# yangdongchao/Text-to-sound-Synthesis

Hardware: AMD Instinct MI355X
Metric: 10s clips/sec whole-node, 100-step Diffsound sample + VQ decode + vocoder (higher is better)
Workload: dtype f32 via 2-way fp16 split (3 MFMA passes, fp32 accumulate); 1 GPU; BASELINE configs[2]: full pipeline, batch 64 per GPU, 100 diffusion steps, codebook 256: CLIP text tower -> 19-layer denoiser -> SpecVQGAN decode -> MelGAN 22 kHz; global_batch=64, n_layer=19, parallelism=caption-sharded x1

## Files before the change

text-to-sound-synthesis_amd/csrc/gemm_f16x2_ps.hip:

```cpp
#include <stdlib.h>

#include "common.h"


typedef _Float16 h8 __attribute__((ext_vector_type(8)));
typedef unsigned u32x4 __attribute__((ext_vector_type(4)));
typedef __attribute__((address_space(1))) const void* ds_gptr;
typedef __attribute__((address_space(3))) void* ds_lptr;

#define PS_HLD 32
#define PS_BM 288
#define PS_BN 256
#define PS_LEAD 6
#define PS_GM 4
#define PS_STAGE_BYTES (2 * 2 * (PS_BM + PS_BN) * PS_HLD * 2)
#define PS_VT_BYTES (2 * 2 * PS_BN * 36 * 4)
#define PS_LDS_BYTES (PS_VT_BYTES > PS_STAGE_BYTES ? PS_VT_BYTES : PS_STAGE_BYTES)
#define PS_SIG(q_) ((0x78 >> (2 * (q_))) & 3)

enum { PS_EPI_ROW = 0, PS_EPI_SPLIT = 1, PS_EPI_ATTN = 2 };

template <int EPI, bool NB16>
__global__ __launch_bounds__(512, 1) void ds_gemm_f16x2_ps_kernel(const GemmParams p) {
    extern __shared__ __attribute__((aligned(16))) unsigned char smem_raw[];
    constexpr int BM = PS_BM, BN = PS_BN, HLD = PS_HLD, LEAD = PS_LEAD;
    constexpr int APL = BM * HLD, BPL = BN * HLD, STAGE = 2 * (APL + BPL);
    _Float16* smem = (_Float16*)smem_raw;
    const int tid = threadIdx.x, lane = tid & 63, wave = tid >> 6, l31 = lane & 31, hh = lane >> 5;
    const int wr = wave >> 2, wc = wave & 3;
    const int L = p.rows_per_sample;
    const int tiles_n = p.N / BN, nblk = gridDim.x;
    int bid = blockIdx.x;
// ... 109 lines not shown
            e1[ks] = *(const h8*)(Ec + APL + swz[ks]);                                               \
        }                                                                                            \
    } while (0)
#define PS_READ_B(buf_, s_)                                                                          \
    do {                                                                                             \
        const _Float16* Bc = smem + (buf_) * STAGE + 2 * APL + (wc * 64 + (s_) * 32 + l31) * HLD;    \
        _Pragma("unroll") for (int ks = 0; ks < 2; ++ks) {                                           \
            b0[s_][ks] = *(const h8*)(Bc + swz[ks]);                                                 \
            b1[s_][ks] = *(const h8*)(Bc + BPL + swz[ks]);                                           \
        }                                                                                            \
    } while (0)
#define PS_QUAD(sa_, sb_)                                                                            \
    do {                                                                                             \
        _Pragma("unroll") for (int ks = 0; ks < 2; ++ks) {                                           \
            _Pragma("unroll") for (int ib = 0; ib < 2; ++ib)                                         \
                acc[2 * (sa_) + ib][sb_] = __builtin_amdgcn_mfma_f32_32x32x16_f16(a1[ks][ib], b0[sb_][ks], acc[2 * (sa_) + ib][sb_], 0, 0, 0); \
            _Pragma("unroll") for (int ib = 0; ib < 2; ++ib)                                         \
                acc[2 * (sa_) + ib][sb_] = __builtin_amdgcn_mfma_f32_32x32x16_f16(a0[ks][ib], b1[sb_][ks], acc[2 * (sa_) + ib][sb_], 0, 0, 0); \
            _Pragma("unroll") for (int ib = 0; ib < 2; ++ib)                                         \
                acc[2 * (sa_) + ib][sb_] = __builtin_amdgcn_mfma_f32_32x32x16_f16(a0[ks][ib], b0[sb_][ks], acc[2 * (sa_) + ib][sb_], 0, 0, 0); \
        }                                                                                            \
    } while (0)
#define PS_EXTRA(sb_)                                                                                \
    do {                                                                                             \
        _Pragma("unroll") for (int ks = 0; ks < 2; ++ks) {                                           \
            acc8 = __builtin_amdgcn_mfma_f32_32x32x16_f16(e1[ks], b0[sb_][ks], acc8, 0, 0, 0);       \
            acc8 = __builtin_amdgcn_mfma_f32_32x32x16_f16(e0[ks], b1[sb_][ks], acc8, 0, 0, 0);       \
            acc8 = __builtin_amdgcn_mfma_f32_32x32x16_f16(e0[ks], b0[sb_][ks], acc8, 0, 0, 0);       \
        }                                                                                            \
    } while (0)
#define PS_READ_EB16(buf_)                                                                           \
    do {                                                                                             \
        const _Float16* Bc = smem + (buf_) * STAGE + 2 * APL + ((2 * wc + wr) * 32 + l15) * HLD;     \
        _Pragma("unroll") for (int tt = 0; tt < 2; ++tt) {                                           \
            eb0[tt] = *(const h8*)(Bc + tt * 16 * HLD + swzq);                                       \
            eb1[tt] = *(const h8*)(Bc + BPL + tt * 16 * HLD + swzq);                                 \
        }                                                                                            \
    } while (0)
#define PS_READ_EA16(buf_)                                                                           \
    do {                                                                                             \
        const _Float16* Ec = smem + (buf_) * STAGE + (256 + l15) * HLD;                              \
        ea0 = *(const h8*)(Ec + swzq);                                                               \
        ea1 = *(const h8*)(Ec + APL + swzq);                                                         \
    } while (0)
#define PS_EXTRA16()                                                                                 \
    do {                                                                                             \
        _Pragma("unroll") for (int tt = 0; tt < 2; ++tt) {                                           \
            acc9[tt] = __builtin_amdgcn_mfma_f32_16x16x32_f16(ea1, eb0[tt], acc9[tt], 0, 0, 0);      \
            acc9[tt] = __builtin_amdgcn_mfma_f32_16x16x32_f16(ea0, eb1[tt], acc9[tt], 0, 0, 0);      \
            acc9[tt] = __builtin_amdgcn_mfma_f32_16x16x32_f16(ea0, eb0[tt], acc9[tt], 0, 0, 0);      \
        }                                                                                            \
    } while (0)
#define PS_PHASE(P, BUF)                                                                             \
    do {                                                                                             \
        if (P == 0) { PS_READ_A(BUF, 0); PS_READ_B(BUF, 0); }                                        \
        if (P == 1) { PS_READ_B(BUF, 1); if (NB16) PS_READ_EB16(BUF); }                              \
        if (P == 2) { PS_READ_A(BUF, 1); if (NB16) PS_READ_EA16(BUF); }                              \
        if (P == 3 && !NB16) PS_READ_E(BUF);                                                         \
        PS_FENCE();                                                                                  \
        {                                                                                            \
            constexpr int dq = (P) + LEAD;                                     \
            const int tq = t + (dq >> 2);                                                            \
            if (tq < nk) {                                                                           \
                PS_ISSUE_LOOP(tq, dq & 3, ((BUF) + (dq >> 2)) & 1);                                  \
                asm volatile("s_waitcnt vmcnt(9)" ::: "memory");    \
// ... 33 lines not shown
        PS_PHASE(0, 1); PS_PHASE(1, 1); PS_PHASE(2, 1); PS_PHASE(3, 1);
        --t;
    }
    if (wr == 0) PS_LBAR();
    asm volatile("s_waitcnt vmcnt(0)" ::: "memory");

    constexpr int WROW = 128, EROW0 = 256;
    constexpr bool HALF_TILE = false;
    const bool hasE = true;
    const int pos0 = 0, tile_rows = L;
#include "gemm_f16x2_ps_epilogue.inc"
}

#define PH_AROWS 144
#define PH_STAGE_BYTES (2 * (PH_AROWS + PS_BN) * PS_HLD * 2)
#define PH_LDS_BYTES (3 * PH_STAGE_BYTES > PS_VT_BYTES ? 3 * PH_STAGE_BYTES : PS_VT_BYTES)

template <int EPI>
__global__ __launch_bounds__(512, 1) void ds_gemm_f16x2_ph_kernel(const GemmParams p) {
    extern __shared__ __attribute__((aligned(16))) unsigned char smem_raw[];
    constexpr bool NB16 = true;
    constexpr int BN = PS_BN, HLD = PS_HLD;
    constexpr int APL = PH_AROWS * HLD, BPL = BN * HLD, STAGE = 2 * (APL + BPL);
    _Float16* smem = (_Float16*)smem_raw;
    const int tid = threadIdx.x, lane = tid & 63, wave = tid >> 6, l31 = lane & 31, hh = lane >> 5;
    const int wr = wave >> 2, wc = wave & 3;
    const int L = p.rows_per_sample;
    const int tiles_n = p.N / BN, nblk = gridDim.x;
    int bid = blockIdx.x;
    {
        const int xcd = bid & 7, idx = bid >> 3, q = nblk >> 3, r = nblk & 7;
// ... 103 lines not shown
        _Pragma("unroll") for (int tt = 0; tt < 2; ++tt) {                                           \
            eb0[tt] = *(const h8*)(Bc + tt * 16 * HLD + swzq);                                       \
            eb1[tt] = *(const h8*)(Bc + BPL + tt * 16 * HLD + swzq);                                 \
        }                                                                                            \
    } while (0)
#define PH_READ_EA16(st_)                                                                            \
    do {                                                                                             \
        const _Float16* Ec = smem + (st_) * STAGE + (128 + l15) * HLD;                               \
        ea0 = *(const h8*)(Ec + swzq);                                                               \
        ea1 = *(const h8*)(Ec + APL + swzq);                                                         \
    } while (0)
#define PH_QUAD(sb_)                                                                                 \
    do {                                                                                             \
        _Pragma("unroll") for (int ks = 0; ks < 2; ++ks) {                                           \
            _Pragma("unroll") for (int ib = 0; ib < 2; ++ib)                                         \
                acc[ib][sb_] = __builtin_amdgcn_mfma_f32_32x32x16_f16(a1[ks][ib], b0[sb_][ks], acc[ib][sb_], 0, 0, 0); \
            _Pragma("unroll") for (int ib = 0; ib < 2; ++ib)                                         \
                acc[ib][sb_] = __builtin_amdgcn_mfma_f32_32x32x16_f16(a0[ks][ib], b1[sb_][ks], acc[ib][sb_], 0, 0, 0); \
            _Pragma("unroll") for (int ib = 0; ib < 2; ++ib)                                         \
                acc[ib][sb_] = __builtin_amdgcn_mfma_f32_32x32x16_f16(a0[ks][ib], b0[sb_][ks], acc[ib][sb_], 0, 0, 0); \
        }                                                                                            \
    } while (0)
#define PH_EXTRA16()                                                                                 \
    do {                                                                                             \
        _Pragma("unroll") for (int tt = 0; tt < 2; ++tt) {                                           \
            acc9[tt] = __builtin_amdgcn_mfma_f32_16x16x32_f16(ea1, eb0[tt], acc9[tt], 0, 0, 0);      \
            acc9[tt] = __builtin_amdgcn_mfma_f32_16x16x32_f16(ea0, eb1[tt], acc9[tt], 0, 0, 0);      \
            acc9[tt] = __builtin_amdgcn_mfma_f32_16x16x32_f16(ea0, eb0[tt], acc9[tt], 0, 0, 0);      \
        }                                                                                            \
    } while (0)
#define PH_PHASE(P, ST)                                                                              \
    do {                                                                                             \
        if (P == 0) { PH_READ_A(ST); PH_READ_B(ST, 0); if (hasE && wr == 0) PH_READ_EB16(ST); }      \
        else { PH_READ_B(ST, 1); if (hasE) { PH_READ_EA16(ST); if (wr == 1) PH_READ_EB16(ST); } }    \
        PS_FENCE();                                                                                  \
        if (tt + 2 < nk) {                                                                           \
            PH_ISSUE_LOOP(P, ((ST) + 2) % 3);                                                        \
            if (P == 0) asm volatile("s_waitcnt vmcnt(11)" ::: "memory");    \
            else asm volatile("s_waitcnt vmcnt(10)" ::: "memory");           \
        } else {                                                                                     \
            asm volatile("s_waitcnt vmcnt(0)" ::: "memory");     \
        }                                                                                            \
        PS_BAR();                                                                                    \
// ... 28 lines not shown
        if (t + 1 < nk) { const int tt = t + 1; PH_PHASE(0, 1); PH_PHASE(1, 1); }
        if (t + 2 < nk) { const int tt = t + 2; PH_PHASE(0, 2); PH_PHASE(1, 2); }
    }
    if (wr == 0) PS_BAR();
    asm volatile("s_waitcnt vmcnt(0)" ::: "memory");
    constexpr int WROW = 64, EROW0 = 128;
    constexpr bool HALF_TILE = true;
#include "gemm_f16x2_ps_epilogue.inc"
}

static bool ps_serves(const GemmParams& p, bool half) {
    const int L = p.rows_per_sample;
    if (!p.a_split || L <= 0 || L > PS_BM - 15 || L <= 240 || p.M % L != 0) return false;
    if (half && L != PS_BM - 16) return false;
    if (p.N % PS_BN != 0 || p.K % 64 != 0 || p.lda != p.K || p.ldw != p.K) return false;
    if (p.store == DS_STORE_ROW && !p.c_split) {
        if (((p.N | p.ldc | p.ldr) & 3) != 0 || (((uintptr_t)p.C | (uintptr_t)p.R) & 15) != 0) return false;
    } else if (p.store == DS_STORE_ROW) {
        if (p.R) return false;
    } else if (p.store == DS_STORE_ATTN) {
        if (p.row_off != 0 || p.attn_heads * 64 % PS_BN != 0) return false;
    } else {
        return false;
    }
    return true;
}

int ds_gemm_f16x2_ps_choice(long B, long N, bool half_ok) {
    const long tf = B * (N / PS_BN), th = 2 * tf;
    const double ef = (double)tf / (double)(((tf + 255) / 256) * 256);
// ... 64 lines not shown
```

text-to-sound-synthesis_amd/csrc/gemm_f16x2_ps_epilogue.inc:

```
    int tid_e = tid;
    asm volatile("" : "+v"(tid_e));
    const int l31e = tid_e & 31, hhe = (tid_e >> 5) & 1, wre = tid_e >> 8, wce = (tid_e >> 6) & 3;
    const int off = row_lo - m0;
    int vhi = off + tile_rows;
    if (vhi > p.M - m0) vhi = p.M - m0;
    const float osc = p.out_scale;
    constexpr bool ALLV = NB16;
    const int qe = (tid_e >> 4) & 3, ne = tid_e & 15;
    const int cl0 = (wce * 2 + 0) * 32 + l31e, cl1 = (wce * 2 + 1) * 32 + l31e;
    const int cl9 = (wce * 2 + wre) * 32 + (NB16 ? PS_SIG(ne >> 2) * 4 + (ne & 3) : l31e);
    float bv0 = 0.f, bv1 = 0.f, bv9a = 0.f, bv9b = 0.f;
    if (p.bias) {
        bv0 = p.bias[n0 + cl0]; bv1 = p.bias[n0 + cl1]; bv9a = p.bias[n0 + cl9];
        if (NB16) bv9b = p.bias[n0 + cl9 + 16];
    }
    constexpr int EBUF = 64 * BN;
#define PS_TROW(S, rs_) ((S) < 4 ? ((rs_) >> 5) * WROW + (S) * 32 + ((rs_) & 31) : EROW0 + (rs_))
#define PS_STEP_VALUES(S, GELU, STORE)                                                               \
    do {                                                                                             \
        if ((S) < 4) {                                                                               \
            _Pragma("unroll") for (int j = 0; j < 2; ++j) {                                          \
                const int cl = j ? cl1 : cl0;                                                        \
                const float bv = j ? bv1 : bv0;                                                      \
                _Pragma("unroll") for (int r = 0; r < 16; ++r) {                                     \
                    float v = acc[(S) < 4 ? (S) : 0][j][r] * osc + bv;                               \
                    if (GELU) v = ds_gelu2_fast(v);                                                  \
                    STORE(wre * 32 + (r & 3) + 8 * (r >> 2) + 4 * hhe, cl, v);                       \
                }                                                                                    \
            }                                                                                        \
        } else if (NB16) {                                                                           \
            _Pragma("unroll") for (int tt = 0; tt < 2; ++tt)                                         \
                _Pragma("unroll") for (int r = 0; r < 4; ++r) {                                      \
                    float v = acc9[tt][r] * osc + (tt ? bv9b : bv9a);                                \
                    if (GELU) v = ds_gelu2_fast(v);                                                  \
                    STORE(4 * PS_SIG(qe) + r, cl9 + tt * 16, v);                                     \
                }                                                                                    \
        } else {                                                                                     \
            _Pragma("unroll") for (int r = 0; r < 16; ++r) {                                         \
                float v = acc8[r] * osc + bv9a;                                                      \
                if (GELU) v = ds_gelu2_fast(v);                                                      \
                STORE((r & 3) + 8 * (r >> 2) + 4 * hhe, cl9, v);                                     \
            }                                                                                        \
        }                                                                                            \
    } while (0)
    const bool gelu = p.act == DS_ACT_GELU2;
    __syncthreads();

    if constexpr (EPI == PS_EPI_ROW) {
#define PS_ST_F32(rs_, cl_, v_) Tf[(rs_) * BN + (cl_)] = (v_)
#define PS_ROW_ITERS(S) (((S) < 4 ? 64 : (NB16 ? 16 : 32)) / 8)
#define PS_ROW_CONST(S, it) ((S) < 4 ? ((it) >> 2) * WROW + (S) * 32 + 8 * ((it) & 3) : EROW0 + 8 * (it))
#define PS_ROW_LOAD(S, res_, HASR)                                                                   \
    do {                                                                                             \
        _Pragma("unroll") for (int it = 0; it < PS_ROW_ITERS(S); ++it) {                             \
            res_[it] = f32x4{0.f, 0.f, 0.f, 0.f};                                                    \
            if (ALLV) {                                                                              \
                if (HASR) res_[it] = *(const f32x4*)(p.R + (size_t)(m0 + PS_ROW_CONST(S, it)) * p.ldr + n0 + voR); \
            } else {                                                                                 \
                const int trow = PS_TROW(S, (tid_e >> 6) + 8 * it);                                  \
                if ((HASR) && trow >= off && trow < vhi)                                             \
                    res_[it] = *(const f32x4*)(p.R + (size_t)(m0 + trow) * p.ldr + n0 + (tid_e & 63) * 4); \
            }                                                                                        \
        }                                                                                            \
    } while (0)
#define PS_ROW_STAGE(S, res_, HASR)                                                                    \
    do {                                                                                             \
        float* Tf = (float*)smem_raw + ((S) & 1) * EBUF;                                             \
        if (!AHEAD) PS_ROW_LOAD(S, res_, HASR);                                                      \
        if (gelu) PS_STEP_VALUES(S, true, PS_ST_F32); else PS_STEP_VALUES(S, false, PS_ST_F32);      \
    } while (0)
#define PS_ROW_STORE(S, res_)                                                                        \
    do {                                                                                             \
        const float* Tf = (const float*)smem_raw + ((S) & 1) * EBUF;                                 \
        const int cc = tid_e & 63, col = n0 + cc * 4;                                                \
        __syncthreads();                                                                             \
        _Pragma("unroll") for (int it = 0; it < PS_ROW_ITERS(S); ++it) {                             \
            const int rs = (tid_e >> 6) + 8 * it, trow = PS_TROW(S, rs);                             \
            if (ALLV || (trow >= off && trow < vhi)) {                                               \
                const f32x4 vv_ = *(const f32x4*)(Tf + rs * BN + cc * 4) + res_[it];                 \
                if (ALLV) *(f32x4*)(p.C + (size_t)(m0 + PS_ROW_CONST(S, it)) * p.ldc + n0 + voC) = vv_; \
                else *(f32x4*)(p.C + (size_t)(m0 + trow) * p.ldc + col) = vv_;                       \
            }                                                                                        \
        }                                                                                            \
    } while (0)
#define PS_ROW_STEP(S, res_, HASR) do { PS_ROW_STAGE(S, res_, HASR); PS_ROW_STORE(S, res_); } while (0)
        f32x4 resA[8], resB[8];
        constexpr bool AHEAD = ALLV;
        const unsigned voR = (unsigned)(tid_e >> 6) * (unsigned)p.ldr + (unsigned)(tid_e & 63) * 4u;
        const unsigned voC = (unsigned)(tid_e >> 6) * (unsigned)p.ldc + (unsigned)(tid_e & 63) * 4u;
#define PS_ROW_ALL(HASR)                                                                             \
    do {                                                                                             \
        if constexpr (!HALF_TILE) {                                                                  \
            if (AHEAD) PS_ROW_LOAD(0, resA, HASR);                                                   \
            PS_ROW_STAGE(0, resA, HASR);                                                             \
            if (AHEAD) PS_ROW_LOAD(1, resB, HASR);                                                   \
            PS_ROW_STORE(0, resA);                                                                   \
            if (AHEAD) PS_ROW_LOAD(2, resA, HASR);                                                   \
            PS_ROW_STEP(1, resB, HASR);                                                              \
            if (AHEAD) PS_ROW_LOAD(3, resB, HASR);                                                   \
            PS_ROW_STEP(2, resA, HASR);                                                              \
            if (AHEAD) PS_ROW_LOAD(4, resA, HASR);                                                   \
            PS_ROW_STEP(3, resB, HASR);                                                              \
            PS_ROW_STEP(4, resA, HASR);                                                              \
        } else {                                                                                     \
            if (AHEAD) PS_ROW_LOAD(0, resA, HASR);                                                   \
            PS_ROW_STAGE(0, resA, HASR);                                                             \
            if (AHEAD) PS_ROW_LOAD(1, resB, HASR);                                                   \
            PS_ROW_STORE(0, resA);                                                                   \
            if (hasE) {                                                                              \
                if (AHEAD) PS_ROW_LOAD(4, resA, HASR);                                               \
                PS_ROW_STEP(1, resB, HASR);                                                          \
                PS_ROW_STEP(4, resA, HASR);                                                          \
            } else {                                                                                 \
                PS_ROW_STEP(1, resB, HASR);                                                          \
            }                                                                                        \
        }                                                                                            \
    } while (0)
        if constexpr (ALLV) {
            if (p.R) PS_ROW_ALL(true); else PS_ROW_ALL(false);
        } else {
            PS_ROW_ALL(p.R != nullptr);
        }
    } else {
#define PS_PACK(v_, dst_) do { dst_ = ds_split_pack(v_); } while (0)
#define PS_ST_SPLIT(rs_, cl_, v_) PS_PACK(v_, T[(rs_) * BN + (cl_)])
#define PS_UNZIP(x_, hi_, lo_)                                                                       \
    do {                                                                                             \
        _Pragma("unroll") for (int e = 0; e < 4; ++e) {           \
            hi_[e] = __builtin_amdgcn_perm((x_)[2 * e + 1], (x_)[2 * e], 0x05040100u);               \
            lo_[e] = __builtin_amdgcn_perm((x_)[2 * e + 1], (x_)[2 * e], 0x07060302u);               \
        }                                                                                            \
    } while (0)
        const int hw = p.attn_heads * 64;
        const int which = EPI == PS_EPI_ATTN ? n0 / hw : 0;
        const int b = tm_;
#define PS_SPLIT_STEP(S)                                                                             \
    do {                                                                                             \
        constexpr int rows_ = (S) < 4 ? 64 : (NB16 ? 16 : 32);                                       \
        constexpr int iters_ = rows_ / 16;                                          \
        unsigned* T = (unsigned*)smem_raw + ((S) & 1) * EBUF;                                        \
        if (gelu) PS_STEP_VALUES(S, true, PS_ST_SPLIT); else PS_STEP_VALUES(S, false, PS_ST_SPLIT);  \
        __syncthreads();                                                                             \
        const int cc = tid_e & 31, col = n0 + cc * 8;                                                \
        _Pragma("unroll") for (int it = 0; it < iters_; ++it) {                                      \
            const int rs = (tid_e >> 5) + 16 * it, trow = PS_TROW(S, rs);                            \
            if (ALLV || (trow >= off && trow < vhi)) {                                               \
                const int row = m0 + trow;                                                           \
                unsigned x[8];                                                                       \
                u32x4 vh, vl;                                                                        \
                *(u32x4*)(x) = *(const u32x4*)(T + rs * BN + cc * 8);                                \
                *(u32x4*)(x + 4) = *(const u32x4*)(T + rs * BN + cc * 8 + 4);                        \
                PS_UNZIP(x, vh, vl);                                                                 \
                _Float16 *d0, *d1;                                                                   \
                if (EPI == PS_EPI_SPLIT) {                                                           \
                    d0 = (_Float16*)p.C + ds_packed_off(row, col, p.ldc >> 5);                       \
                    d1 = d0 + p.c_plane;                                                             \
                } else {                                                                             \
                    const int pos = trow - off + pos0;                                               \
                    const int hc = col - which * hw, head = hc >> 6, d = hc & 63;                    \
                    const size_t bh = (size_t)b * p.attn_heads + head;                               \
                    if (which == 0) {                                                                \
                        d0 = (_Float16*)p.C + (bh * L + pos) * 64 + d;                               \
                        d1 = d0 + p.attn_qplane;                                                     \
                    } else {                                                                         \
                        d0 = (_Float16*)p.attn_kv + (bh * 4) * ((size_t)p.attn_nkey * 64) + ds_attn_k_off(pos, d); \
                        d1 = d0 + (size_t)p.attn_nkey * 64;                                          \
                    }                                                                                \
                }                                                                                    \
                *(u32x4*)d0 = vh;                                                                    \
                *(u32x4*)d1 = vl;                                                                    \
            }                                                                                        \
        }                                                                                            \
    } while (0)
        constexpr int VLD = 36, VGRP = BN * VLD;
#define PS_VT_STAGE(S, GELU)                                                                         \
    do {                                                                                             \
        unsigned* T2 = (unsigned*)smem_raw + ((S) & 1) * (2 * VGRP);                                 \
        if ((S) < 4) {                                                                               \
            _Pragma("unroll") for (int j = 0; j < 2; ++j)                                            \
                _Pragma("unroll") for (int q = 0; q < 4; ++q) {                                      \
                    u32x4 w;                                                                         \
                    _Pragma("unroll") for (int e = 0; e < 4; ++e) {                                  \
                        float v = acc[(S) < 4 ? (S) : 0][j][4 * q + e] * osc + (j ? bv1 : bv0);      \
                        if (GELU) v = ds_gelu2_fast(v);                                              \
                        PS_PACK(v, w[e]);                                                            \
                    }                                                                                \
                    *(u32x4*)(T2 + wre * VGRP + (j ? cl1 : cl0) * VLD + 8 * q + 4 * hhe) = w;        \
                }                                                                                    \
        } else if (NB16) {                                                                           \
            _Pragma("unroll") for (int tt = 0; tt < 2; ++tt) {                                       \
                u32x4 w;                                                                             \
                _Pragma("unroll") for (int e = 0; e < 4; ++e) {                                      \
                    float v = acc9[tt][e] * osc + (tt ? bv9b : bv9a);                                \
                    if (GELU) v = ds_gelu2_fast(v);                                                  \
                    PS_PACK(v, w[e]);                                                                \
                }                                                                                    \
                *(u32x4*)(T2 + (cl9 + tt * 16) * VLD + 4 * PS_SIG(qe)) = w;                          \
            }                                                                                        \
        } else {                                                                                     \
            _Pragma("unroll") for (int q = 0; q < 4; ++q) {                                          \
                u32x4 w;                                                                             \
                _Pragma("unroll") for (int e = 0; e < 4; ++e) {                                      \
                    float v = acc8[4 * q + e] * osc + bv9a;                                          \
                    if (GELU) v = ds_gelu2_fast(v);                                                  \
                    PS_PACK(v, w[e]);                                                                \
                }                                                                                    \
                *(u32x4*)(T2 + cl9 * VLD + 8 * q + 4 * hhe) = w;                                     \
            }                                                                                        \
        }                                                                                            \
    } while (0)
#define PS_VT_STEP(S)                                                                                \
    do {                                                                                             \
        constexpr int ngrp_ = (S) < 4 ? 2 : 1;                                                       \
        constexpr int grows_ = (S) < 4 ? 32 : (NB16 ? 16 : 32);                                      \
        const unsigned* T2 = (const unsigned*)smem_raw + ((S) & 1) * (2 * VGRP);                     \
        if (gelu) PS_VT_STAGE(S, true); else PS_VT_STAGE(S, false);                                  \
        __syncthreads();                                                                             \
        const int pln = p.attn_nkey * 64;                                                            \
        _Pragma("unroll") for (int g = 0; g < ngrp_; ++g) {                                          \
            const int G0 = (S) < 4 ? g * WROW + (S) * 32 : EROW0;    \
            const int lo = ALLV || G0 > off ? G0 : off;                                              \
            const int hi = ALLV || G0 + grows_ < vhi ? G0 + grows_ : vhi;                            \
            if (!ALLV && lo >= hi) continue;                                                         \
            const unsigned* Tg = T2 + g * VGRP;                                                      \
            if (ALLV || (lo == G0 && hi == G0 + grows_ && ((G0 - off) & 7) == 0)) {                  \
                constexpr int upc_ = grows_ / 8;                        \
                constexpr int iters_ = BN * upc_ / 512;                                   \
                _Pragma("unroll") for (int it = 0; it < iters_; ++it) {                              \
                    const int task = tid_e + 512 * it, cl = task / upc_, u = task % upc_;            \
                    const int hc = n0 + cl - 2 * hw, head = hc >> 6, d = hc & 63;                    \
                    _Float16* img = (_Float16*)p.attn_kv + (((size_t)b * p.attn_heads + head) * 4 + 2) * (size_t)pln; \
                    unsigned x[8];                                                                   \
                    *(u32x4*)(x) = *(const u32x4*)(Tg + cl * VLD + 8 * u);                           \
                    *(u32x4*)(x + 4) = *(const u32x4*)(Tg + cl * VLD + 8 * u + 4);                   \
                    u32x4 vh, vl;                                                                    \
                    PS_UNZIP(x, vh, vl);                                                             \
                    _Float16* dst = img + ds_attn_vt_off(G0 - off + pos0 + 8 * u, d, p.attn_nkey);   \
                    *(u32x4*)dst = vh;                                                               \
                    *(u32x4*)(dst + pln) = vl;                                                       \
                }                                                                                    \
            } else {                                                                                 \
                const int u_first = (lo - off) >> 3, units = ((hi - off + 7) >> 3) - u_first;        \
                const int cl = tid_e & (BN - 1);                                                     \
                const int hc = n0 + cl - 2 * hw, head = hc >> 6, d = hc & 63;                        \
                _Float16* img = (_Float16*)p.attn_kv + (((size_t)b * p.attn_heads + head) * 4 + 2) * (size_t)pln; \
                for (int u = tid_e >> 8; u < units; u += 2) {                                        \
                    const int k0 = (u_first + u) * 8;                     \
                    const int r0 = k0 + off - G0;                    \
                    _Float16* dst = img + ds_attn_vt_off(k0 + pos0, d, p.attn_nkey);                 \
                    if (r0 >= lo - G0 && r0 + 8 <= hi - G0) {        \
                        unsigned x[8];                                                               \
                        _Pragma("unroll") for (int e = 0; e < 8; ++e) x[e] = Tg[cl * VLD + r0 + e];  \
                        u32x4 vh, vl;                                                                \
                        PS_UNZIP(x, vh, vl);                                                         \
                        *(u32x4*)dst = vh;                                                           \
                        *(u32x4*)(dst + pln) = vl;                                                   \
                    } else {                                                                         \
                        _Pragma("unroll") for (int e = 0; e < 8; ++e)                                \
                            if (r0 + e >= lo - G0 && r0 + e < hi - G0) {                             \
                                const unsigned x1 = Tg[cl * VLD + r0 + e];                           \
                                dst[e] = __builtin_bit_cast(_Float16, (unsigned short)(x1 & 0xffffu)); \
                                dst[pln + e] = __builtin_bit_cast(_Float16, (unsigned short)(x1 >> 16)); \
                            }                                                                        \
                    }                                                                                \
                }                                                                                    \
            }                                                                                        \
        }                                                                                            \
    } while (0)
        if (EPI == PS_EPI_ATTN && which == 2) {
            if constexpr (!HALF_TILE) {
                PS_VT_STEP(0); PS_VT_STEP(1); PS_VT_STEP(2); PS_VT_STEP(3); PS_VT_STEP(4);
            } else {
                PS_VT_STEP(0); PS_VT_STEP(1);
                if (hasE) PS_VT_STEP(4);
            }
        } else {
            if constexpr (!HALF_TILE) {
                PS_SPLIT_STEP(0); PS_SPLIT_STEP(1); PS_SPLIT_STEP(2); PS_SPLIT_STEP(3); PS_SPLIT_STEP(4);
            } else {
                PS_SPLIT_STEP(0); PS_SPLIT_STEP(1);
                if (hasE) PS_SPLIT_STEP(4);
            }
        }
    }
#undef PS_TROW
#undef PS_STEP_VALUES
#undef PS_ST_F32
#undef PS_ROW_STEP
#undef PS_ROW_ALL
#undef PS_ROW_STAGE
#undef PS_ROW_STORE
#undef PS_ROW_LOAD
#undef PS_ROW_ITERS
#undef PS_ROW_CONST
#undef PS_PACK
#undef PS_ST_SPLIT
#undef PS_UNZIP
#undef PS_SPLIT_STEP
#undef PS_VT_STAGE
#undef PS_VT_STEP
```

Measured before the change: 22.63 clips/s.

## Transpose MFMA operands and restructure GEMM epilogue around quad stores

Swaps the A/B operand order in every MFMA so each lane's accumulator holds four contiguous output columns instead of rows. The epilogue then writes raw f32x4 quads into a padded LDS tile (BN+4) and applies scale, bias and GELU at readout, with bias loaded as vectors. A new direct split-store path (on by default for the SPLIT epilogue) writes results without the LDS round trip. The aim is to cut scalar LDS stores, per-element bias loads and epilogue shared-memory traffic. In exchange it adds a bias-alignment gate that can send unaligned cases to a fallback path, and it is a large macro rewrite with layout-correctness risk.

Result: faster. 23.01 clips/s (median of 6 runs) (+1.7%).

```diff
diff --git a/text-to-sound-synthesis_amd/csrc/gemm_f16x2_ps.hip b/text-to-sound-synthesis_amd/csrc/gemm_f16x2_ps.hip
--- a/text-to-sound-synthesis_amd/csrc/gemm_f16x2_ps.hip
+++ b/text-to-sound-synthesis_amd/csrc/gemm_f16x2_ps.hip
@@ -5,6 +5,7 @@
 
 typedef _Float16 h8 __attribute__((ext_vector_type(8)));
 typedef unsigned u32x4 __attribute__((ext_vector_type(4)));
+typedef unsigned u32x2 __attribute__((ext_vector_type(2)));
 typedef __attribute__((address_space(1))) const void* ds_gptr;
 typedef __attribute__((address_space(3))) void* ds_lptr;
 
@@ -14,8 +15,14 @@
 #define PS_LEAD 6
 #define PS_GM 4
 #define PS_STAGE_BYTES (2 * 2 * (PS_BM + PS_BN) * PS_HLD * 2)
-#define PS_VT_BYTES (2 * 2 * PS_BN * 36 * 4)
-#define PS_LDS_BYTES (PS_VT_BYTES > PS_STAGE_BYTES ? PS_VT_BYTES : PS_STAGE_BYTES)
+#define PS_EPI_BYTES (2 * 64 * (PS_BN + 4) * 4)
+#ifndef PS_DIRECT_SPLIT
+#define PS_DIRECT_SPLIT 1
+#endif
+#ifndef PS_DIRECT_QK
+#define PS_DIRECT_QK 0
+#endif
+#define PS_LDS_BYTES (PS_EPI_BYTES > PS_STAGE_BYTES ? PS_EPI_BYTES : PS_STAGE_BYTES)
 #define PS_SIG(q_) ((0x78 >> (2 * (q_))) & 3)
 
 enum { PS_EPI_ROW = 0, PS_EPI_SPLIT = 1, PS_EPI_ATTN = 2 };
@@ -155,19 +162,19 @@
     do {                                                                                             \
         _Pragma("unroll") for (int ks = 0; ks < 2; ++ks) {                                           \
             _Pragma("unroll") for (int ib = 0; ib < 2; ++ib)                                         \
-                acc[2 * (sa_) + ib][sb_] = __builtin_amdgcn_mfma_f32_32x32x16_f16(a1[ks][ib], b0[sb_][ks], acc[2 * (sa_) + ib][sb_], 0, 0, 0); \
+                acc[2 * (sa_) + ib][sb_] = __builtin_amdgcn_mfma_f32_32x32x16_f16(b0[sb_][ks], a1[ks][ib], acc[2 * (sa_) + ib][sb_], 0, 0, 0); \
             _Pragma("unroll") for (int ib = 0; ib < 2; ++ib)                                         \
-                acc[2 * (sa_) + ib][sb_] = __builtin_amdgcn_mfma_f32_32x32x16_f16(a0[ks][ib], b1[sb_][ks], acc[2 * (sa_) + ib][sb_], 0, 0, 0); \
+                acc[2 * (sa_) + ib][sb_] = __builtin_amdgcn_mfma_f32_32x32x16_f16(b1[sb_][ks], a0[ks][ib], acc[2 * (sa_) + ib][sb_], 0, 0, 0); \
             _Pragma("unroll") for (int ib = 0; ib < 2; ++ib)                                         \
-                acc[2 * (sa_) + ib][sb_] = __builtin_amdgcn_mfma_f32_32x32x16_f16(a0[ks][ib], b0[sb_][ks], acc[2 * (sa_) + ib][sb_], 0, 0, 0); \
+                acc[2 * (sa_) + ib][sb_] = __builtin_amdgcn_mfma_f32_32x32x16_f16(b0[sb_][ks], a0[ks][ib], acc[2 * (sa_) + ib][sb_], 0, 0, 0); \
         }                                                                                            \
     } while (0)
 #define PS_EXTRA(sb_)                                                                                \
     do {                                                                                             \
         _Pragma("unroll") for (int ks = 0; ks < 2; ++ks) {                                           \
-            acc8 = __builtin_amdgcn_mfma_f32_32x32x16_f16(e1[ks], b0[sb_][ks], acc8, 0, 0, 0);       \
-            acc8 = __builtin_amdgcn_mfma_f32_32x32x16_f16(e0[ks], b1[sb_][ks], acc8, 0, 0, 0);       \
-            acc8 = __builtin_amdgcn_mfma_f32_32x32x16_f16(e0[ks], b0[sb_][ks], acc8, 0, 0, 0);       \
+            acc8 = __builtin_amdgcn_mfma_f32_32x32x16_f16(b0[sb_][ks], e1[ks], acc8, 0, 0, 0);       \
+            acc8 = __builtin_amdgcn_mfma_f32_32x32x16_f16(b1[sb_][ks], e0[ks], acc8, 0, 0, 0);       \
+            acc8 = __builtin_amdgcn_mfma_f32_32x32x16_f16(b0[sb_][ks], e0[ks], acc8, 0, 0, 0);       \
         }                                                                                            \
     } while (0)
 #define PS_READ_EB16(buf_)                                                                           \
@@ -187,9 +194,9 @@
 #define PS_EXTRA16()                                                                                 \
     do {                                                                                             \
         _Pragma("unroll") for (int tt = 0; tt < 2; ++tt) {                                           \
-            acc9[tt] = __builtin_amdgcn_mfma_f32_16x16x32_f16(ea1, eb0[tt], acc9[tt], 0, 0, 0);      \
-            acc9[tt] = __builtin_amdgcn_mfma_f32_16x16x32_f16(ea0, eb1[tt], acc9[tt], 0, 0, 0);      \
-            acc9[tt] = __builtin_amdgcn_mfma_f32_16x16x32_f16(ea0, eb0[tt], acc9[tt], 0, 0, 0);      \
+            acc9[tt] = __builtin_amdgcn_mfma_f32_16x16x32_f16(eb0[tt], ea1, acc9[tt], 0, 0, 0);      \
+            acc9[tt] = __builtin_amdgcn_mfma_f32_16x16x32_f16(eb1[tt], ea0, acc9[tt], 0, 0, 0);      \
+            acc9[tt] = __builtin_amdgcn_mfma_f32_16x16x32_f16(eb0[tt], ea0, acc9[tt], 0, 0, 0);      \
         }                                                                                            \
     } while (0)
 #define PS_PHASE(P, BUF)                                                                             \
@@ -253,7 +260,7 @@
 
 #define PH_AROWS 144
 #define PH_STAGE_BYTES (2 * (PH_AROWS + PS_BN) * PS_HLD * 2)
-#define PH_LDS_BYTES (3 * PH_STAGE_BYTES > PS_VT_BYTES ? 3 * PH_STAGE_BYTES : PS_VT_BYTES)
+#define PH_LDS_BYTES (3 * PH_STAGE_BYTES > PS_EPI_BYTES ? 3 * PH_STAGE_BYTES : PS_EPI_BYTES)
 
 template <int EPI>
 __global__ __launch_bounds__(512, 1) void ds_gemm_f16x2_ph_kernel(const GemmParams p) {
@@ -387,19 +394,19 @@
     do {                                                                                             \
         _Pragma("unroll") for (int ks = 0; ks < 2; ++ks) {                                           \
             _Pragma("unroll") for (int ib = 0; ib < 2; ++ib)                                         \
-                acc[ib][sb_] = __builtin_amdgcn_mfma_f32_32x32x16_f16(a1[ks][ib], b0[sb_][ks], acc[ib][sb_], 0, 0, 0); \
+                acc[ib][sb_] = __builtin_amdgcn_mfma_f32_32x32x16_f16(b0[sb_][ks], a1[ks][ib], acc[ib][sb_], 0, 0, 0); \
             _Pragma("unroll") for (int ib = 0; ib < 2; ++ib)                                         \
-                acc[ib][sb_] = __builtin_amdgcn_mfma_f32_32x32x16_f16(a0[ks][ib], b1[sb_][ks], acc[ib][sb_], 0, 0, 0); \
+                acc[ib][sb_] = __builtin_amdgcn_mfma_f32_32x32x16_f16(b1[sb_][ks], a0[ks][ib], acc[ib][sb_], 0, 0, 0); \
             _Pragma("unroll") for (int ib = 0; ib < 2; ++ib)                                         \
-                acc[ib][sb_] = __builtin_amdgcn_mfma_f32_32x32x16_f16(a0[ks][ib], b0[sb_][ks], acc[ib][sb_], 0, 0, 0); \
+                acc[ib][sb_] = __builtin_amdgcn_mfma_f32_32x32x16_f16(b0[sb_][ks], a0[ks][ib], acc[ib][sb_], 0, 0, 0); \
         }                                                                                            \
     } while (0)
 #define PH_EXTRA16()                                                                                 \
     do {                                                                                             \
         _Pragma("unroll") for (int tt = 0; tt < 2; ++tt) {                                           \
-            acc9[tt] = __builtin_amdgcn_mfma_f32_16x16x32_f16(ea1, eb0[tt], acc9[tt], 0, 0, 0);      \
-            acc9[tt] = __builtin_amdgcn_mfma_f32_16x16x32_f16(ea0, eb1[tt], acc9[tt], 0, 0, 0);      \
-            acc9[tt] = __builtin_amdgcn_mfma_f32_16x16x32_f16(ea0, eb0[tt], acc9[tt], 0, 0, 0);      \
+            acc9[tt] = __builtin_amdgcn_mfma_f32_16x16x32_f16(eb0[tt], ea1, acc9[tt], 0, 0, 0);      \
+            acc9[tt] = __builtin_amdgcn_mfma_f32_16x16x32_f16(eb1[tt], ea0, acc9[tt], 0, 0, 0);      \
+            acc9[tt] = __builtin_amdgcn_mfma_f32_16x16x32_f16(eb0[tt], ea0, acc9[tt], 0, 0, 0);      \
         }                                                                                            \
     } while (0)
 #define PH_PHASE(P, ST)                                                                              \
@@ -458,6 +465,7 @@
     if (!p.a_split || L <= 0 || L > PS_BM - 15 || L <= 240 || p.M % L != 0) return false;
     if (half && L != PS_BM - 16) return false;
     if (p.N % PS_BN != 0 || p.K % 64 != 0 || p.lda != p.K || p.ldw != p.K) return false;
+    if (((uintptr_t)p.bias & 15) != 0) return false;
     if (p.store == DS_STORE_ROW && !p.c_split) {
         if (((p.N | p.ldc | p.ldr) & 3) != 0 || (((uintptr_t)p.C | (uintptr_t)p.R) & 15) != 0) return false;
     } else if (p.store == DS_STORE_ROW) {
diff --git a/text-to-sound-synthesis_amd/csrc/gemm_f16x2_ps_epilogue.inc b/text-to-sound-synthesis_amd/csrc/gemm_f16x2_ps_epilogue.inc
--- a/text-to-sound-synthesis_amd/csrc/gemm_f16x2_ps_epilogue.inc
+++ b/text-to-sound-synthesis_amd/csrc/gemm_f16x2_ps_epilogue.inc
@@ -7,47 +7,42 @@
     const float osc = p.out_scale;
     constexpr bool ALLV = NB16;
     const int qe = (tid_e >> 4) & 3, ne = tid_e & 15;
-    const int cl0 = (wce * 2 + 0) * 32 + l31e, cl1 = (wce * 2 + 1) * 32 + l31e;
-    const int cl9 = (wce * 2 + wre) * 32 + (NB16 ? PS_SIG(ne >> 2) * 4 + (ne & 3) : l31e);
-    float bv0 = 0.f, bv1 = 0.f, bv9a = 0.f, bv9b = 0.f;
-    if (p.bias) {
-        bv0 = p.bias[n0 + cl0]; bv1 = p.bias[n0 + cl1]; bv9a = p.bias[n0 + cl9];
-        if (NB16) bv9b = p.bias[n0 + cl9 + 16];
-    }
-    constexpr int EBUF = 64 * BN;
+    const int cb0 = (wce * 2 + 0) * 32, cb1 = (wce * 2 + 1) * 32, cb9 = (wce * 2 + wre) * 32;
+    const int cq = 4 * hhe, cq9 = NB16 ? 4 * PS_SIG(qe) : cq;
+    const int r9 = NB16 ? 4 * PS_SIG(ne >> 2) + (ne & 3) : l31e;
+    const bool hasb = p.bias != nullptr;
+    const float* bsrc = (hasb ? p.bias : (const float*)p.W) + n0;
+#define PS_BIAS4(col_) (hasb ? *(const f32x4*)(bsrc + (col_)) : f32x4{0.f, 0.f, 0.f, 0.f})
+#define PS_BIAS1(col_) (hasb ? bsrc[col_] : 0.f)
+#define PS_FIN(x_, b_, GELU, t_)                                                                     \
+    do {                                                                                             \
+        t_ = (x_) * osc + (b_);                                                                      \
+        if (GELU) t_ = ds_gelu2_fast(t_);                                                            \
+    } while (0)
+    constexpr int ELD = BN + 4, EBUF = 64 * ELD;
 #define PS_TROW(S, rs_) ((S) < 4 ? ((rs_) >> 5) * WROW + (S) * 32 + ((rs_) & 31) : EROW0 + (rs_))
-#define PS_STEP_VALUES(S, GELU, STORE)                                                               \
+#define PS_STEP_QUADS(S, STORE4)                                                                     \
     do {                                                                                             \
         if ((S) < 4) {                                                                               \
-            _Pragma("unroll") for (int j = 0; j < 2; ++j) {                                          \
-                const int cl = j ? cl1 : cl0;                                                        \
-                const float bv = j ? bv1 : bv0;                                                      \
-                _Pragma("unroll") for (int r = 0; r < 16; ++r) {                                     \
-                    float v = acc[(S) < 4 ? (S) : 0][j][r] * osc + bv;                               \
-                    if (GELU) v = ds_gelu2_fast(v);                                                  \
-                    STORE(wre * 32 + (r & 3) + 8 * (r >> 2) + 4 * hhe, cl, v);                       \
+            _Pragma("unroll") for (int j = 0; j < 2; ++j)                                            \
+                _Pragma("unroll") for (int qd = 0; qd < 4; ++qd) {                                   \
+                    const f32x16& A_ = acc[(S) < 4 ? (S) : 0][j];                                    \
+                    STORE4(wre * 32 + l31e, (j ? cb1 : cb0) + 8 * qd + cq,                           \
+                           (f32x4{A_[4 * qd], A_[4 * qd + 1], A_[4 * qd + 2], A_[4 * qd + 3]}));     \
                 }                                                                                    \
-            }                                                                                        \
         } else if (NB16) {                                                                           \
-            _Pragma("unroll") for (int tt = 0; tt < 2; ++tt)                                         \
-                _Pragma("unroll") for (int r = 0; r < 4; ++r) {                                      \
-                    float v = acc9[tt][r] * osc + (tt ? bv9b : bv9a);                                \
-                    if (GELU) v = ds_gelu2_fast(v);                                                  \
-                    STORE(4 * PS_SIG(qe) + r, cl9 + tt * 16, v);                                     \
-                }                                                                                    \
+            _Pragma("unroll") for (int tt = 0; tt < 2; ++tt) STORE4(r9, cb9 + 16 * tt + cq9, acc9[tt]); \
         } else {                                                                                     \
-            _Pragma("unroll") for (int r = 0; r < 16; ++r) {                                         \
-                float v = acc8[r] * osc + bv9a;                                                      \
-                if (GELU) v = ds_gelu2_fast(v);                                                      \
-                STORE((r & 3) + 8 * (r >> 2) + 4 * hhe, cl9, v);                                     \
-            }                                                                                        \
-        }                                                                                            \
-    } while (0)
+            _Pragma("unroll") for (int qd = 0; qd < 4; ++qd)                                         \
+                STORE4(r9, cb9 + 8 * qd + cq9,                                                       \
+                       (f32x4{acc8[4 * qd], acc8[4 * qd + 1], acc8[4 * qd + 2], acc8[4 * qd + 3]})); \
+        }                                                                                            \
+    } while (0)
+#define PS_ST_RAW(rs_, cl_, v_) *(f32x4*)(Tf + (rs_) * ELD + (cl_)) = (v_)
     const bool gelu = p.act == DS_ACT_GELU2;
     __syncthreads();
 
     if constexpr (EPI == PS_EPI_ROW) {
-#define PS_ST_F32(rs_, cl_, v_) Tf[(rs_) * BN + (cl_)] = (v_)
 #define PS_ROW_ITERS(S) (((S) < 4 ? 64 : (NB16 ? 16 : 32)) / 8)
 #define PS_ROW_CONST(S, it) ((S) < 4 ? ((it) >> 2) * WROW + (S) * 32 + 8 * ((it) & 3) : EROW0 + 8 * (it))
 #define PS_ROW_LOAD(S, res_, HASR)                                                                   \
@@ -63,13 +58,13 @@
             }                                                                                        \
         }                                                                                            \
     } while (0)
-#define PS_ROW_STAGE(S, res_, HASR)                                                                    \
+#define PS_ROW_STAGE(S, res_, HASR)                                                                  \
     do {                                                                                             \
         float* Tf = (float*)smem_raw + ((S) & 1) * EBUF;                                             \
         if (!AHEAD) PS_ROW_LOAD(S, res_, HASR);                                                      \
-        if (gelu) PS_STEP_VALUES(S, true, PS_ST_F32); else PS_STEP_VALUES(S, false, PS_ST_F32);      \
-    } while (0)
-#define PS_ROW_STORE(S, res_)                                                                        \
+        PS_STEP_QUADS(S, PS_ST_RAW);                                                                 \
+    } while (0)
+#define PS_ROW_STORE(S, res_, HASR)                                                                  \
     do {                                                                                             \
         const float* Tf = (const float*)smem_raw + ((S) & 1) * EBUF;                                 \
         const int cc = tid_e & 63, col = n0 + cc * 4;                                                \
@@ -77,14 +72,19 @@
         _Pragma("unroll") for (int it = 0; it < PS_ROW_ITERS(S); ++it) {                             \
             const int rs = (tid_e >> 6) + 8 * it, trow = PS_TROW(S, rs);                             \
             if (ALLV || (trow >= off && trow < vhi)) {                                               \
-                const f32x4 vv_ = *(const f32x4*)(Tf + rs * BN + cc * 4) + res_[it];                 \
+                const f32x4 xx_ = *(const f32x4*)(Tf + rs * ELD + cc * 4);                           \
+                f32x4 vv_;                                                                           \
+                if (gelu) { _Pragma("unroll") for (int e = 0; e < 4; ++e) PS_FIN(xx_[e], bias4[e], true, vv_[e]); } \
+                else { _Pragma("unroll") for (int e = 0; e < 4; ++e) PS_FIN(xx_[e], bias4[e], false, vv_[e]); }    \
+                if (HASR) vv_ += res_[it];               \
                 if (ALLV) *(f32x4*)(p.C + (size_t)(m0 + PS_ROW_CONST(S, it)) * p.ldc + n0 + voC) = vv_; \
                 else *(f32x4*)(p.C + (size_t)(m0 + trow) * p.ldc + col) = vv_;                       \
             }                                                                                        \
         }                                                                                            \
     } while (0)
-#define PS_ROW_STEP(S, res_, HASR) do { PS_ROW_STAGE(S, res_, HASR); PS_ROW_STORE(S, res_); } while (0)
+#define PS_ROW_STEP(S, res_, HASR) do { PS_ROW_STAGE(S, res_, HASR); PS_ROW_STORE(S, res_, HASR); } while (0)
         f32x4 resA[8], resB[8];
+        const f32x4 bias4 = PS_BIAS4((tid_e & 63) * 4);
         constexpr bool AHEAD = ALLV;
         const unsigned voR = (unsigned)(tid_e >> 6) * (unsigned)p.ldr + (unsigned)(tid_e & 63) * 4u;
         const unsigned voC = (unsigned)(tid_e >> 6) * (unsigned)p.ldc + (unsigned)(tid_e & 63) * 4u;
@@ -94,7 +94,7 @@
             if (AHEAD) PS_ROW_LOAD(0, resA, HASR);                                                   \
             PS_ROW_STAGE(0, resA, HASR);                                                             \
             if (AHEAD) PS_ROW_LOAD(1, resB, HASR);                                                   \
-            PS_ROW_STORE(0, resA);                                                                   \
+            PS_ROW_STORE(0, resA, HASR);                                                             \
             if (AHEAD) PS_ROW_LOAD(2, resA, HASR);                                                   \
             PS_ROW_STEP(1, resB, HASR);                                                              \
             if (AHEAD) PS_ROW_LOAD(3, resB, HASR);                                                   \
@@ -106,7 +106,7 @@
             if (AHEAD) PS_ROW_LOAD(0, resA, HASR);                                                   \
             PS_ROW_STAGE(0, resA, HASR);                                                             \
             if (AHEAD) PS_ROW_LOAD(1, resB, HASR);                                                   \
-            PS_ROW_STORE(0, resA);                                                                   \
+            PS_ROW_STORE(0, resA, HASR);                                                             \
             if (hasE) {                                                                              \
                 if (AHEAD) PS_ROW_LOAD(4, resA, HASR);                                               \
                 PS_ROW_STEP(1, resB, HASR);                                                          \
@@ -123,7 +123,6 @@
         }
     } else {
 #define PS_PACK(v_, dst_) do { dst_ = ds_split_pack(v_); } while (0)
-#define PS_ST_SPLIT(rs_, cl_, v_) PS_PACK(v_, T[(rs_) * BN + (cl_)])
 #define PS_UNZIP(x_, hi_, lo_)                                                                       \
     do {                                                                                             \
         _Pragma("unroll") for (int e = 0; e < 4; ++e) {           \
@@ -134,87 +133,138 @@
         const int hw = p.attn_heads * 64;
         const int which = EPI == PS_EPI_ATTN ? n0 / hw : 0;
         const int b = tm_;
+#define PS_QUAD_SPLIT(A_, r0_, bq_, GELU, h_, l_)                                                    \
+    do {                                                                                             \
+        unsigned x_[4];                                                                              \
+        _Pragma("unroll") for (int e = 0; e < 4; ++e) {                                              \
+            float t_;                                                                                \
+            PS_FIN((A_)[(r0_) + e], (bq_)[e], GELU, t_);                                             \
+            PS_PACK(t_, x_[e]);                                                                      \
+        }                                                                                            \
+        h_[0] = __builtin_amdgcn_perm(x_[1], x_[0], 0x05040100u);                                    \
+        h_[1] = __builtin_amdgcn_perm(x_[3], x_[2], 0x05040100u);                                    \
+        l_[0] = __builtin_amdgcn_perm(x_[1], x_[0], 0x07060302u);                                    \
+        l_[1] = __builtin_amdgcn_perm(x_[3], x_[2], 0x07060302u);                                    \
+    } while (0)
+#define PS_SWAP(a_, b_, o0_, o1_)                                                                    \
+    do {                                                                                             \
+        const auto sw_ = __builtin_amdgcn_permlane32_swap(a_, b_, false, false);                     \
+        o0_ = sw_[0];                                                                                \
+        o1_ = sw_[1];                                                                                \
+    } while (0)
+#define PS_DST(trow_, tcol_, d0_, d1_)                                                               \
+    do {                                                                                             \
+        const int row = m0 + (trow_), col = n0 + (tcol_);                                            \
+        if (EPI == PS_EPI_SPLIT) {                                                                   \
+            d0_ = (_Float16*)p.C + ds_packed_off(row, col, p.ldc >> 5);                              \
+            d1_ = d0_ + p.c_plane;                                                                   \
+        } else {                                                                                     \
+            const int pos = (trow_) - off + pos0;                                                    \
+            const int hc = col - which * hw, head = hc >> 6, d = hc & 63;                            \
+            const size_t bh = (size_t)b * p.attn_heads + head;                                       \
+            if (which == 0) {                                                                        \
+                d0_ = (_Float16*)p.C + (bh * L + pos) * 64 + d;                                      \
+                d1_ = d0_ + p.attn_qplane;                                                           \
+            } else {                                                                                 \
+                d0_ = (_Float16*)p.attn_kv + (bh * 4) * ((size_t)p.attn_nkey * 64) + ds_attn_k_off(pos, d); \
+                d1_ = d0_ + (size_t)p.attn_nkey * 64;                                                \
+            }                                                                                        \
+        }                                                                                            \
+    } while (0)
+#define PS_DIRECT_BLOCK(A_, trow_, cb_, bqs_, GELU)                                                  \
+    do {                                                                                             \
+        const int trw_ = (trow_);                                                                    \
+        const bool ok_ = ALLV || (trw_ >= off && trw_ < vhi);                                        \
+        _Pragma("unroll") for (int m = 0; m < 2; ++m) {                                              \
+            unsigned hA[2], lA[2], hB[2], lB[2];                                                     \
+            u32x4 vh, vl;                                                                            \
+            PS_QUAD_SPLIT(A_, 8 * m, (bqs_)[2 * m], GELU, hA, lA);                                   \
+            PS_QUAD_SPLIT(A_, 8 * m + 4, (bqs_)[2 * m + 1], GELU, hB, lB);                           \
+            PS_SWAP(hA[0], hB[0], vh[0], vh[2]);                                                     \
+            PS_SWAP(hA[1], hB[1], vh[1], vh[3]);                                                     \
+            PS_SWAP(lA[0], lB[0], vl[0], vl[2]);                                                     \
+            PS_SWAP(lA[1], lB[1], vl[1], vl[3]);                                                     \
+            if (ok_) {                                                                               \
+                _Float16 *d0, *d1;                                                                   \
+                PS_DST(trw_, (cb_) + 16 * m + 8 * hhe, d0, d1);                                      \
+                *(u32x4*)d0 = vh;                                                                    \
+                *(u32x4*)d1 = vl;                                                                    \
+            }                                                                                        \
+        }                                                                                            \
+    } while (0)
+#define PS_DIRECT_STEP_G(S, GELU)                                                                    \
+    do {                                                                                             \
+        if ((S) < 4) {                                                                               \
+            PS_DIRECT_BLOCK(acc[(S) < 4 ? (S) : 0][0], wre * WROW + (S) * 32 + l31e, cb0, bqd[0], GELU); \
+            PS_DIRECT_BLOCK(acc[(S) < 4 ? (S) : 0][1], wre * WROW + (S) * 32 + l31e, cb1, bqd[1], GELU); \
+        } else if (NB16) {                                   \
+            _Pragma("unroll") for (int tt = 0; tt < 2; ++tt) {                                       \
+                unsigned h9[2], l9[2];                                                               \
+                _Float16 *d0, *d1;                                                                   \
+                PS_QUAD_SPLIT(acc9[tt], 0, bqd[2][tt], GELU, h9, l9);                                \
+                PS_DST(EROW0 + r9, cb9 + 16 * tt + cq9, d0, d1);                                     \
+                *(u32x2*)d0 = u32x2{h9[0], h9[1]};                                                   \
+                *(u32x2*)d1 = u32x2{l9[0], l9[1]};                                                   \
+            }                                                                                        \
+        } else {                                                                                     \
+            PS_DIRECT_BLOCK(acc8, EROW0 + r9, cb9, bqd[2], GELU);                                    \
+        }                                                                                            \
+    } while (0)
+#define PS_DIRECT_STEP(S) do { if (gelu) PS_DIRECT_STEP_G(S, true); else PS_DIRECT_STEP_G(S, false); } while (0)
+#define PS_DIRECT_BIAS()                                                                             \
+    f32x4 bqd[3][4];                                                                                 \
+    _Pragma("unroll") for (int qd = 0; qd < 4; ++qd) {                                               \
+        bqd[0][qd] = PS_BIAS4(cb0 + 8 * qd + cq);                                                    \
+        bqd[1][qd] = PS_BIAS4(cb1 + 8 * qd + cq);                                                    \
+        bqd[2][qd] = NB16 ? PS_BIAS4(cb9 + 16 * (qd & 1) + cq9) : PS_BIAS4(cb9 + 8 * qd + cq9);      \
+    }
+#define PS_FIN_SPLIT8(xf_, b8_, x_)                                                                  \
+    do {                                                                                             \
+        _Pragma("unroll") for (int e = 0; e < 8; ++e) {                                              \
+            float t_;                                                                                \
+            if (gelu) PS_FIN((xf_)[e], (b8_)[e], true, t_); else PS_FIN((xf_)[e], (b8_)[e], false, t_); \
+            PS_PACK(t_, x_[e]);                                                                      \
+        }                                                                                            \
+    } while (0)
 #define PS_SPLIT_STEP(S)                                                                             \
     do {                                                                                             \
         constexpr int rows_ = (S) < 4 ? 64 : (NB16 ? 16 : 32);                                       \
         constexpr int iters_ = rows_ / 16;                                          \
-        unsigned* T = (unsigned*)smem_raw + ((S) & 1) * EBUF;                                        \
-        if (gelu) PS_STEP_VALUES(S, true, PS_ST_SPLIT); else PS_STEP_VALUES(S, false, PS_ST_SPLIT);  \
+        float* Tf = (float*)smem_raw + ((S) & 1) * EBUF;                                             \
+        PS_STEP_QUADS(S, PS_ST_RAW);                                                                 \
         __syncthreads();                                                                             \
-        const int cc = tid_e & 31, col = n0 + cc * 8;                                                \
+        const int cc = tid_e & 31;                                                                   \
         _Pragma("unroll") for (int it = 0; it < iters_; ++it) {                                      \
             const int rs = (tid_e >> 5) + 16 * it, trow = PS_TROW(S, rs);                            \
             if (ALLV || (trow >= off && trow < vhi)) {                                               \
-                const int row = m0 + trow;                                                           \
+                float xf[8];                                                                         \
                 unsigned x[8];                                                                       \
                 u32x4 vh, vl;                                                                        \
-                *(u32x4*)(x) = *(const u32x4*)(T + rs * BN + cc * 8);                                \
-                *(u32x4*)(x + 4) = *(const u32x4*)(T + rs * BN + cc * 8 + 4);                        \
+                *(f32x4*)(xf) = *(const f32x4*)(Tf + rs * ELD + cc * 8);                             \
+                *(f32x4*)(xf + 4) = *(const f32x4*)(Tf + rs * ELD + cc * 8 + 4);                     \
+                PS_FIN_SPLIT8(xf, bias8, x);                                                         \
                 PS_UNZIP(x, vh, vl);                                                                 \
                 _Float16 *d0, *d1;                                                                   \
-                if (EPI == PS_EPI_SPLIT) {                                                           \
-                    d0 = (_Float16*)p.C + ds_packed_off(row, col, p.ldc >> 5);                       \
-                    d1 = d0 + p.c_plane;                                                             \
-                } else {                                                                             \
-                    const int pos = trow - off + pos0;                                               \
-                    const int hc = col - which * hw, head = hc >> 6, d = hc & 63;                    \
-                    const size_t bh = (size_t)b * p.attn_heads + head;                               \
-                    if (which == 0) {                                                                \
-                        d0 = (_Float16*)p.C + (bh * L + pos) * 64 + d;                               \
-                        d1 = d0 + p.attn_qplane;                                                     \
-                    } else {                                                                         \
-                        d0 = (_Float16*)p.attn_kv + (bh * 4) * ((size_t)p.attn_nkey * 64) + ds_attn_k_off(pos, d); \
-                        d1 = d0 + (size_t)p.attn_nkey * 64;                                          \
-                    }                                                                                \
-                }                                                                                    \
+                PS_DST(trow, cc * 8, d0, d1);                                                        \
                 *(u32x4*)d0 = vh;                                                                    \
                 *(u32x4*)d1 = vl;                                                                    \
             }                                                                                        \
         }                                                                                            \
     } while (0)
-        constexpr int VLD = 36, VGRP = BN * VLD;
-#define PS_VT_STAGE(S, GELU)                                                                         \
-    do {                                                                                             \
-        unsigned* T2 = (unsigned*)smem_raw + ((S) & 1) * (2 * VGRP);                                 \
-        if ((S) < 4) {                                                                               \
-            _Pragma("unroll") for (int j = 0; j < 2; ++j)                                            \
-                _Pragma("unroll") for (int q = 0; q < 4; ++q) {                                      \
-                    u32x4 w;                                                                         \
-                    _Pragma("unroll") for (int e = 0; e < 4; ++e) {                                  \
-                        float v = acc[(S) < 4 ? (S) : 0][j][4 * q + e] * osc + (j ? bv1 : bv0);      \
-                        if (GELU) v = ds_gelu2_fast(v);                                              \
-                        PS_PACK(v, w[e]);                                                            \
-                    }                                                                                \
-                    *(u32x4*)(T2 + wre * VGRP + (j ? cl1 : cl0) * VLD + 8 * q + 4 * hhe) = w;        \
-                }                                                                                    \
-        } else if (NB16) {                                                                           \
-            _Pragma("unroll") for (int tt = 0; tt < 2; ++tt) {                                       \
-                u32x4 w;                                                                             \
-                _Pragma("unroll") for (int e = 0; e < 4; ++e) {                                      \
-                    float v = acc9[tt][e] * osc + (tt ? bv9b : bv9a);                                \
-                    if (GELU) v = ds_gelu2_fast(v);                                                  \
-                    PS_PACK(v, w[e]);                                                                \
-                }                                                                                    \
-                *(u32x4*)(T2 + (cl9 + tt * 16) * VLD + 4 * PS_SIG(qe)) = w;                          \
-            }                                                                                        \
-        } else {                                                                                     \
-            _Pragma("unroll") for (int q = 0; q < 4; ++q) {                                          \
-                u32x4 w;                                                                             \
-                _Pragma("unroll") for (int e = 0; e < 4; ++e) {                                      \
-                    float v = acc8[4 * q + e] * osc + bv9a;                                          \
-                    if (GELU) v = ds_gelu2_fast(v);                                                  \
-                    PS_PACK(v, w[e]);                                                                \
-                }                                                                                    \
-                *(u32x4*)(T2 + cl9 * VLD + 8 * q + 4 * hhe) = w;                                     \
-            }                                                                                        \
-        }                                                                                            \
+#define PS_VT_W(g_, r_, cl_) T2[((g_) * 32 + (r_)) * ELD + ((cl_) ^ ((((r_) >> 4) & 1) << 4))]
+#define PS_ST_VT(rs_, cl_, v_) *(f32x4*)&PS_VT_W(0, rs_, cl_) = (v_)
+#define PS_VT_UNIT(g_, r0_, cl_, bv_, x_)                                                            \
+    do {                                                                                             \
+        float xf_[8], b8_[8];                                                                        \
+        _Pragma("unroll") for (int e = 0; e < 8; ++e) { xf_[e] = PS_VT_W(g_, (r0_) + e, cl_); b8_[e] = (bv_); } \
+        PS_FIN_SPLIT8(xf_, b8_, x_);                                                                 \
     } while (0)
 #define PS_VT_STEP(S)                                                                                \
     do {                                                                                             \
         constexpr int ngrp_ = (S) < 4 ? 2 : 1;                                                       \
         constexpr int grows_ = (S) < 4 ? 32 : (NB16 ? 16 : 32);                                      \
-        const unsigned* T2 = (const unsigned*)smem_raw + ((S) & 1) * (2 * VGRP);                     \
-        if (gelu) PS_VT_STAGE(S, true); else PS_VT_STAGE(S, false);                                  \
+        float* T2 = (float*)smem_raw + ((S) & 1) * EBUF;                                             \
+        PS_STEP_QUADS(S, PS_ST_VT);                                                                  \
         __syncthreads();                                                                             \
         const int pln = p.attn_nkey * 64;                                                            \
         _Pragma("unroll") for (int g = 0; g < ngrp_; ++g) {                                          \
@@ -222,7 +272,6 @@
             const int lo = ALLV || G0 > off ? G0 : off;                                              \
             const int hi = ALLV || G0 + grows_ < vhi ? G0 + grows_ : vhi;                            \
             if (!ALLV && lo >= hi) continue;                                                         \
-            const unsigned* Tg = T2 + g * VGRP;                                                      \
             if (ALLV || (lo == G0 && hi == G0 + grows_ && ((G0 - off) & 7) == 0)) {                  \
                 constexpr int upc_ = grows_ / 8;                        \
                 constexpr int iters_ = BN * upc_ / 512;                                   \
@@ -231,8 +280,7 @@
                     const int hc = n0 + cl - 2 * hw, head = hc >> 6, d = hc & 63;                    \
                     _Float16* img = (_Float16*)p.attn_kv + (((size_t)b * p.attn_heads + head) * 4 + 2) * (size_t)pln; \
                     unsigned x[8];                                                                   \
-                    *(u32x4*)(x) = *(const u32x4*)(Tg + cl * VLD + 8 * u);                           \
-                    *(u32x4*)(x + 4) = *(const u32x4*)(Tg + cl * VLD + 8 * u + 4);                   \
+                    PS_VT_UNIT(g, 8 * u, cl, upc_ == 4 ? bvt[it] : bvt[2], x);                                    \
                     u32x4 vh, vl;                                                                    \
                     PS_UNZIP(x, vh, vl);                                                             \
                     _Float16* dst = img + ds_attn_vt_off(G0 - off + pos0 + 8 * u, d, p.attn_nkey);   \
@@ -250,7 +298,7 @@
                     _Float16* dst = img + ds_attn_vt_off(k0 + pos0, d, p.attn_nkey);                 \
                     if (r0 >= lo - G0 && r0 + 8 <= hi - G0) {        \
                         unsigned x[8];                                                               \
-                        _Pragma("unroll") for (int e = 0; e < 8; ++e) x[e] = Tg[cl * VLD + r0 + e];  \
+                        PS_VT_UNIT(g, r0, cl, bvt[3], x);                                    \
                         u32x4 vh, vl;                                                                \
                         PS_UNZIP(x, vh, vl);                                                         \
                         *(u32x4*)dst = vh;                                                           \
@@ -258,7 +306,10 @@
                     } else {                                                                         \
                         _Pragma("unroll") for (int e = 0; e < 8; ++e)                                \
                             if (r0 + e >= lo - G0 && r0 + e < hi - G0) {                             \
-                                const unsigned x1 = Tg[cl * VLD + r0 + e];                           \
+                                float t1;                                                            \
+                                if (gelu) PS_FIN(PS_VT_W(g, r0 + e, cl), bvt[3], true, t1);   \
+                                else PS_FIN(PS_VT_W(g, r0 + e, cl), bvt[3], false, t1);       \
+                                const unsigned x1 = ds_split_pack(t1);                               \
                                 dst[e] = __builtin_bit_cast(_Float16, (unsigned short)(x1 & 0xffffu)); \
                                 dst[pln + e] = __builtin_bit_cast(_Float16, (unsigned short)(x1 >> 16)); \
                             }                                                                        \
@@ -268,6 +319,8 @@
         }                                                                                            \
     } while (0)
         if (EPI == PS_EPI_ATTN && which == 2) {
+            const float bvt[4] = {PS_BIAS1(tid_e >> 2), PS_BIAS1((tid_e >> 2) + 128), PS_BIAS1(tid_e >> 1),
+                                  PS_BIAS1(tid_e & (BN - 1))};
             if constexpr (!HALF_TILE) {
                 PS_VT_STEP(0); PS_VT_STEP(1); PS_VT_STEP(2); PS_VT_STEP(3); PS_VT_STEP(4);
             } else {
@@ -275,17 +328,37 @@
                 if (hasE) PS_VT_STEP(4);
             }
         } else {
-            if constexpr (!HALF_TILE) {
-                PS_SPLIT_STEP(0); PS_SPLIT_STEP(1); PS_SPLIT_STEP(2); PS_SPLIT_STEP(3); PS_SPLIT_STEP(4);
+            constexpr bool DIRECT = EPI == PS_EPI_SPLIT ? PS_DIRECT_SPLIT : PS_DIRECT_QK;
+            if constexpr (DIRECT) {
+                PS_DIRECT_BIAS();
+                if constexpr (!HALF_TILE) {
+                    PS_DIRECT_STEP(0); PS_DIRECT_STEP(1); PS_DIRECT_STEP(2); PS_DIRECT_STEP(3); PS_DIRECT_STEP(4);
+                } else {
+                    PS_DIRECT_STEP(0); PS_DIRECT_STEP(1);
+                    if (hasE) PS_DIRECT_STEP(4);
+                }
             } else {
-                PS_SPLIT_STEP(0); PS_SPLIT_STEP(1);
-                if (hasE) PS_SPLIT_STEP(4);
+                float bias8[8];
+                *(f32x4*)bias8 = PS_BIAS4((tid_e & 31) * 8);
+                *(f32x4*)(bias8 + 4) = PS_BIAS4((tid_e & 31) * 8 + 4);
+                if constexpr (!HALF_TILE) {
+                    PS_SPLIT_STEP(0); PS_SPLIT_STEP(1); PS_SPLIT_STEP(2); PS_SPLIT_STEP(3); PS_SPLIT_STEP(4);
+                } else {
+                    PS_SPLIT_STEP(0); PS_SPLIT_STEP(1);
+                    if (hasE) PS_SPLIT_STEP(4);
+                }
             }
         }
     }
 #undef PS_TROW
-#undef PS_STEP_VALUES
-#undef PS_ST_F32
+#undef PS_STEP_QUADS
+#undef PS_BIAS4
+#undef PS_BIAS1
+#undef PS_FIN
+#undef PS_ST_RAW
+#undef PS_FIN_SPLIT8
+#undef PS_VT_UNIT
+#undef PS_DIRECT_BIAS
 #undef PS_ROW_STEP
 #undef PS_ROW_ALL
 #undef PS_ROW_STAGE
@@ -294,8 +367,14 @@
 #undef PS_ROW_ITERS
 #undef PS_ROW_CONST
 #undef PS_PACK
-#undef PS_ST_SPLIT
+#undef PS_QUAD_SPLIT
+#undef PS_SWAP
+#undef PS_DST
+#undef PS_DIRECT_BLOCK
+#undef PS_DIRECT_STEP_G
+#undef PS_ST_VT
 #undef PS_UNZIP
+#undef PS_DIRECT_STEP
 #undef PS_SPLIT_STEP
-#undef PS_VT_STAGE
+#undef PS_VT_W
 #undef PS_VT_STEP
```
